# chairclr/PathTracing

Hardware: AMD Instinct MI355X
Metric: Mrays/s (higher is better)
Workload: dtype f32

## Files before the change

pathtracing_amd/csrc/frame.cpp:

```cpp
#include "scene.h"
#include <hip/hip_runtime.h>
#include <algorithm>
#include <cmath>
#include <cstdio>
#include <cstdlib>
#include <cstring>
#include <vector>

using namespace ptrt;

namespace {

uint32_t host_pcg(uint32_t x)
{
    uint32_t s = x * 747796405u + 2891336453u;
    uint32_t w = ((s >> ((s >> 28) + 4u)) ^ s) * 277803737u;
    return (w >> 22) ^ w;
}

uint32_t faster(double rate_simple, double rate_packed) { return rate_packed > 1.10 * rate_simple ? EXT_PACKED : EXT_SIMPLE; }
struct ExtendFrame {
    ExtendChoice &mem;
    bool undecided;
    uint32_t frame_kernel, kernel;
// ... 18 lines not shown
            kernel = EXT_SIMPLE; mixed = probe_n[1] >= enough / 8u;
        } else kernel = mem.kernel = faster(probe_n[0] / std::max((double)ms_simple, 1e-6), probe_n[1] / std::max((double)ms_packed, 1e-6));
        return hipSuccess;
    }
    void frame_done(uint64_t rays, double gpu_ms, bool cold)
    {
        if (!undecided || mem.kernel != 0u || cold) return;
        if (mixed || rays < (1u << 20) || !(gpu_ms > 0.0)) { if (++mem.misses >= 3u) mem.kernel = EXT_SIMPLE; return; }
        (frame_kernel == EXT_PACKED ? mem.rate_packed : mem.rate_simple) = (double)rays / gpu_ms;
        if (mem.rate_simple > 0.0 && mem.rate_packed > 0.0) mem.kernel = faster(mem.rate_simple, mem.rate_packed);
    }
};

hipEvent_t pool_event(pt_context *c, size_t i)
{
    while (c->ev_pool.size() <= i) {
        Event e;
        if (e.create() != hipSuccess) return nullptr;
        c->ev_pool.push_back(std::move(e));
    }
    return c->ev_pool[i];
}

struct Frame {
    uint32_t nranks, streams, pixel_slots, n_slots, shard_cap, samples_per_stream, lag, n_loops, packed_chunk, default_bounces;
    uint32_t forced;
    bool profile, count, split, bucket, full_state, accumulate, mapped, compact;
    bool nee;
    NeeArgs nee_args;
    bool env;
    EnvArgs env_args;
    Accumulation::Key sums_key;
    size_t q_entries; uint64_t total_spp, allocs_before;
    PathState ps; FrameParams fp;
    uint32_t iters; uint64_t slot_launches; size_t n_events;
    std::vector<uint64_t> trace_alive, trace_rays;
};

}

pt_status FrameTemplate::build_if_differs(pt_context *c, hipStream_t q, Key key, const DeviceScene &ds, const PathState &ps, const FrameParams &fp,
                                          const QueueSizes &sizes)
{
    key.q = q_init.p;
    if (valid && key == key_) return PT_OK;
    valid = false; HIP_TRY(c, hipMemsetAsync(cnt_init.p, 0, sizeof(uint32_t) * kCntTotalWords, q));
    PathState pt = ps; pt.counters = cnt_init.p; pt.q_ext[0] = q_init.p;
    const bool dense = key.first_spp < key.streams;
    HIP_TRY(c, launch_generate(q, ds, pt, fp, dense ? 2u : 0u));
    bound = key.shard_cap;
    if (dense) {
        uint32_t *h = sizes.template_sizes();
        HIP_TRY(c, hipMemcpyAsync(h, cnt_init.p, sizeof(uint32_t) * kShards * kCounterStride, hipMemcpyDeviceToHost, q));
        HIP_TRY(c, hipStreamSynchronize(q));
// ... 68 lines not shown
    if (!f.full_state) HIP_TRY(c, c->start.reserve(f.q_entries));
    const uint32_t ovf = s->tree.stack_overflow();
    if (ovf) HIP_TRY(c, c->stack_ovf.ensure((size_t)ovf * f.q_entries));
    if (f.nee) {
        HIP_TRY(c, c->nee_ext.ensure(f.n_slots)); HIP_TRY(c, c->nee_rad.ensure(f.n_slots));
        f.nee_args = NeeArgs{ s->d_lights.p, s->d_cdf.p, s->d_pa.p, s->n_lights, c->nee_ext.p, c->nee_rad.p };
    }
    if (f.env) f.env_args = s->env.args(f.nee && s->env.lit() && s->n_lights ? 0.5f : 1.0f);
    if (f.nranks == 1) HIP_TRY(c, c->out.resize(p->width, p->height));
    PathState &ps = f.ps;
    ps.ray_o = c->ray_o.p; ps.ray_d = c->ray_d.p; ps.thr = c->thr.p; ps.sd = c->sd.p; ps.acc = c->acc.p; ps.q_ext[0] = c->q_ext0.p; ps.q_ext[1] = c->q_ext1.p;
    if (f.split) { ps.hit = c->hit.p; ps.q_bucket[B_METAL] = c->q_metal.p; ps.q_bucket[B_DIELECTRIC] = c->q_dielectric.p; }
    ps.counters = c->counters.p; ps.stack_ovf = c->stack_ovf.p; ps.stack_ovf_entries = ovf; ps.n_slots = f.n_slots; ps.shard_cap = f.shard_cap;
    ps.shard_base = 0; ps.shard_count = kShards; ps.compact_below = t.compact_below; ps.finish_below = t.finish_below; ps.sparse_below = t.sparse_below;
    ps.repack_sticky = (f.samples_per_stream <= t.sticky_samples && t.compact_below > 0.f) ? 1u : 0u;
    ps.host_ring = c->sizes.begin(f.mapped); ps.ring_slots = kLag;
    f.compact = f.bucket || (ps.repack_sticky && f.samples_per_stream <= 2u);
    FrameParams &fp = f.fp;
    fp.width = p->width; fp.height = p->height; fp.spp = p->spp; fp.max_depth = p->max_depth; fp.rr_start = p->rr_start;
    fp.seed_hashed = host_pcg(p->seed); fp.sample_offset = p->sample_offset; fp.ray_eps = p->ray_eps;
    fp.rank = p->rank; fp.nranks = f.nranks; fp.tiles_x = lay.tiles_x; fp.n_tiles = lay.n_tiles; fp.streams = f.streams; fp.slots_per_stream = f.pixel_slots;
    div_magic(f.streams, fp.streams_magic, fp.streams_shift); div_magic(lay.tiles_x, fp.tiles_x_magic, fp.tiles_x_shift);
    fp.offset_mod = p->sample_offset % f.streams; fp.accumulate = f.accumulate ? 1u : 0u;
    return PT_OK;
}

static pt_status start_frame(pt_context *c, const pt_scene *s, const pt_render_params *p, const Frame &f)
{
    hipStream_t q = c->stream;
    if (f.full_state) {
        HIP_TRY(c, hipMemsetAsync(c->counters.p, 0, sizeof(uint32_t) * kCntTotalWords, q));
        HIP_TRY(c, hipEventRecord(c->ev_start, q));
        HIP_TRY(c, launch_generate(q, s->ds, f.ps, f.fp, 1u));
    } else {
        HIP_TRY(c, hipEventRecord(c->ev_start, q));
        FrameTemplate::Key key{};
        key.w = p->width; key.h = p->height; key.rank = p->rank; key.nranks = f.nranks; key.streams = f.streams; key.first_spp = std::min(p->spp, f.streams);
        key.offset = f.fp.offset_mod; key.n_slots = f.n_slots; key.shard_cap = f.shard_cap; key.acc = c->acc.p;
        const pt_status st = c->start.build_if_differs(c, q, key, s->ds, f.ps, f.fp, c->sizes);
        if (st != PT_OK) return st;
        HIP_TRY(c, hipMemcpyAsync(c->counters.p, c->start.counters(), sizeof(uint32_t) * kCntTotalWords, hipMemcpyDeviceToDevice, q));
    }
    c->start.frame_ran(f.accumulate || f.full_state);
    return PT_OK;
}

static pt_status run_loops(pt_context *c, const pt_scene *s, const pt_render_params *p, Frame &f, ExtendFrame &x)
{
    hipStream_t q = c->stream; const uint32_t n_loops = f.n_loops, per_group = kShards / n_loops;
    struct Loop { hipStream_t stream; uint32_t base, bound, iters; bool done; } loops[kMaxGroups];
    HIP_TRY(c, hipEventRecord(c->ev_fork, q));
    for (uint32_t g = 0; g < n_loops; ++g) {
        loops[g] = Loop{ n_loops == 1 ? q : c->group_stream[g], g * per_group, f.full_state ? f.shard_cap : c->start.first_bound(), 0u, false };
        if (loops[g].stream != q) HIP_TRY(c, hipStreamWaitEvent(loops[g].stream, c->ev_fork, 0));
    }
    const uint64_t max_iters = (uint64_t)p->spp * p->max_depth * (f.nee ? 2u : 1u) + kLag + 2;
    const bool trace = f.profile && getenv("PTRT_TRACE") != nullptr;
    const int shade_mode = (s->has_specular || f.env) ? 2 : 0;
    for (uint32_t live = n_loops; live > 0;) {
        for (uint32_t g = 0; g < n_loops; ++g) {
            Loop &L = loops[g];
            if (L.done) continue;
            if (L.iters >= max_iters) return fail(c, PT_ERR_INTERNAL, "wavefront loop did not drain after %u iterations", L.iters);
            const uint32_t it = L.iters; PathState pg = f.ps; pg.shard_base = L.base; pg.shard_count = per_group;
// ... 46 lines not shown
    if (f.nranks == 1)
        HIP_TRY(c, launch_assemble(q, c->out.tiles.p, 1, f.pixel_slots, p->width, p->height, fp.tiles_x, fp.n_tiles, 1.0f / (float)f.total_spp, c->out.fb.p, c->out.fb8.p));
    HIP_TRY(c, hipEventRecord(c->ev_stop, q));
    HIP_TRY(c, hipMemcpyAsync(c->sizes.frame_end(), c->counters.p, sizeof(uint32_t) * kCntTotalWords, hipMemcpyDeviceToHost, q));
    HIP_TRY(c, hipStreamSynchronize(q));
    pt_stats out{}; const CounterView hc{ c->sizes.frame_end(), 0u };
    if (hc.error()) return fail(c, PT_ERR_INTERNAL, "device error flag 0x%x (1 = traversal stack overflow, 2 = step limit)", hc.error());
    for (uint32_t sh = 0; sh < kShards; ++sh) {
        if (hc.word(cnt_alive_index(0, sh)) || hc.word(cnt_alive_index(1, sh)) || hc.word(cnt_alive_index(2, sh))) return fail(c, PT_ERR_INTERNAL, "extend queue of shard %u not empty at frame end", sh);
        out.rays += hc.u64(cnt_rays_index(sh));
    }
    float ms = 0.f; HIP_TRY(c, hipEventElapsedTime(&ms, c->ev_start, c->ev_stop)); out.gpu_ms = ms;
    out.node_visits = hc.u64(kCntNodes); out.tri_tests = hc.u64(kCntTris); out.sphere_tests = hc.u64(kCntSph);
    out.reserved[3] = (hc.u64(kCntWaveNodeIters) & 0xFFFFFFFFFFull) | (hc.u64(kCntWaveNodeIters + 2) << 40);
    if (f.count && getenv("PTRT_TRACE")) {
        const double slots = 64.0 * (double)hc.u64(kCntWaveNodeIters), v = (double)out.node_visits, lf = (double)hc.u64(kCntIdleLeaf), dn = (double)hc.u64(kCntIdleDone);
        if (slots > 0) fprintf(stderr, "ptrt: node-loop lane-slots %.3g: visiting %.1f %%, waiting at a leaf %.1f %%, ray finished %.1f %%, no ray %.1f %%\n", slots,
                               100 * v / slots, 100 * lf / slots, 100 * dn / slots, 100 * (slots - v - lf - dn) / slots);
    }
    out.iterations = f.iters; out.extend_launches = f.iters;
    x.frame_done(out.rays, out.gpu_ms, g_device_allocs != f.allocs_before);
    out.reserved[0] = x.kernel ? x.kernel : (uint32_t)EXT_SIMPLE;
    out.reserved[1] = hc.word(kCntCompactions);
    uint64_t px = 0;
    for (uint32_t t = p->rank; t < fp.n_tiles; t += f.nranks) {
        const uint32_t tx = t % fp.tiles_x, ty = t / fp.tiles_x;
        px += (uint64_t)std::min(kTile, p->width - tx * kTile) * std::min(kTile, p->height - ty * kTile);
    }
    out.paths = px * p->spp;
    out.reserved[2] = f.slot_launches + px * std::min(f.streams, p->spp);
    if (f.profile) {
        const bool trace = getenv("PTRT_TRACE") != nullptr;
        for (size_t i = 0; i + 2 < f.n_events; i += 3) {
            float a = 0.f, b = 0.f; HIP_TRY(c, hipEventElapsedTime(&a, c->ev_pool[i], c->ev_pool[i + 1]));
            HIP_TRY(c, hipEventElapsedTime(&b, c->ev_pool[i + 1], c->ev_pool[i + 2]));
            out.extend_ms += a; out.shade_ms += b;
            if (trace) fprintf(stderr, "ptrt: iteration %3zu  rays %10llu  alive after %10llu  extend %8.3f ms  shade %8.3f ms\n", i / 3,
                               (unsigned long long)(i / 3 < f.trace_rays.size() ? f.trace_rays[i / 3] : 0),
                               (unsigned long long)(i / 3 < f.trace_alive.size() ? f.trace_alive[i / 3] : 0), a, b);
        }
        out.other_ms = out.gpu_ms - out.extend_ms - out.shade_ms;
    }
    c->out.tiles_hold(f.pixel_slots); c->sums.complete(f.sums_key, f.total_spp);
    if (f.nranks == 1) c->out.complete(FrameOutputs::Holds::path_traced);
    if (stats) *stats = out;
    return PT_OK;
}

static pt_status render_frame(pt_context *c, const pt_scene *s, const pt_render_params *p, pt_stats *stats)
{
    if (!c || !p) return fail(c, PT_ERR_INVALID_ARGUMENT, "pt_render: NULL argument");
    pt_tile_layout lay; pt_status st = layout_of(p, &lay);
    if (st != PT_OK) return fail(c, st, "pt_render: bad width/height/rank/nranks/tile_size");
    HIP_TRY(c, hipSetDevice(c->device));
    c->out.replace();
    if (p->mode == PT_REFERENCE_SPHERE) {
        HIP_TRY(c, c->out.resize(p->width, p->height));
        HIP_TRY(c, hipEventRecord(c->ev_start, c->stream));
        HIP_TRY(c, launch_reference_sphere(c->stream, p->width, p->height, c->out.fb.p, c->out.fb8.p));
        HIP_TRY(c, hipEventRecord(c->ev_stop, c->stream));
        HIP_TRY(c, hipStreamSynchronize(c->stream));
        float ms = 0.f; HIP_TRY(c, hipEventElapsedTime(&ms, c->ev_start, c->ev_stop));
        pt_stats out{};
        out.gpu_ms = ms; out.other_ms = ms; out.rays = out.paths = (uint64_t)p->width * p->height; out.iterations = 1;
// ... 19 lines not shown
```

pathtracing_amd/csrc/kernels.hip:

```cpp
#include "ptrt_internal.h"
#include "pt_device.h"
#include <algorithm>
#include <cstdlib>
#include <type_traits>


using namespace ptd;

namespace ptrt {

PT_DEV uint32_t lane_prefix(uint64_t m) { return __builtin_amdgcn_mbcnt_hi((uint32_t)(m >> 32), __builtin_amdgcn_mbcnt_lo((uint32_t)m, 0u)); }
PT_DEV uint32_t lane_id() { return lane_prefix(~0ull); }

typedef const float4 __attribute__((address_space(4))) *uniform_f4;
PT_DEV uniform_f4 as_uniform(const float4 *p) { return (uniform_f4)(uintptr_t)p; }
PT_DEV float4 uniform_load(uniform_f4 p, uint32_t i) { return make_float4(p[i].x, p[i].y, p[i].z, p[i].w); }
PT_DEV uint32_t spheres_test(const float4 *spheres, uint32_t n_spheres, uint32_t first_id, V3 o, V3 d, Hit &h)
{
    const uniform_f4 sp = as_uniform(spheres);
    for (uint32_t j = 0; j < n_spheres; j += 4u) {
        const float4 s0 = uniform_load(sp, j), s1 = uniform_load(sp, j + 1u), s2 = uniform_load(sp, j + 2u), s3 = uniform_load(sp, j + 3u);
        sphere_test(s0, first_id + j, o, d, h);
        if (j + 1u < n_spheres) sphere_test(s1, first_id + j + 1u, o, d, h);
        if (j + 2u < n_spheres) sphere_test(s2, first_id + j + 2u, o, d, h);
// ... 352 lines not shown
}
PT_DEV void path_init(const DeviceScene &sc, const FrameParams &fp, uint32_t slot, PathRegs &r)
{
    uint32_t x = 0, y = 0;
    slot_pixel(slot, fp, x, y);
    r.sample = first_sample(slot, fp);
    r.key = path_key(fp.seed_hashed, y * fp.width + x, fp.sample_offset + r.sample);
    camera_ray_of(sc.cam, x, y, r.key, r.o, r.d);
    r.T = v3(1.f, 1.f, 1.f);
    r.depth = 0u;
}
template <bool NEE = false>
PT_DEV void path_begin(uint32_t it, uint32_t slot, PathRegs &r, NeeRegs *nr = nullptr)
{
    if (it == 0u) {
        path_init(cold().sc, cold().fp, slot, r);
        if (!cold().fp.accumulate) at(cold().ps.acc, slot) = make_float4(0.f, 0.f, 0.f, 0.f);
    } else {
        const PathState &ps = cold().ps;
        path_load(ps, slot, r);
        if constexpr (NEE) { nr->flags = __float_as_uint(at(ps.ray_o, slot).w); nr->aux = at(ps.ray_d, slot).w; }
    }
}

__global__ void __launch_bounds__(kBlock) k_generate(DeviceScene sc, PathState ps, FrameParams fp, uint32_t full)
{
    uint32_t shard, bx, nbx;
    block_pos(ps, shard, bx, nbx);
    const uint32_t j = bx * kBlock + threadIdx.x;
    const uint32_t t = j >> kShardGroupShift, rot = (shard + kShards - t % kShards) % kShards;
    const uint32_t slot = ((t * kShards + rot) << kShardGroupShift) | (j & ((1u << kShardGroupShift) - 1u));
    uint32_t x = 0, y = 0;
    const bool in_range = j < ps.shard_cap && slot < ps.n_slots;
    const uint32_t first = first_sample(slot, fp);
    const bool valid = in_range && first < fp.spp && slot_pixel(slot, fp, x, y);
    if (in_range && !fp.accumulate) ps.acc[slot] = make_float4(0.f, 0.f, 0.f, 0.f);
    if (valid && full == 1u) {
        PathRegs r;
        path_init(sc, fp, slot, r);
        path_store(ps, slot, r);
    }
    if (full == 2u) wave_push(&ps.counters[cnt_ext_index(0, shard)], ps.q_ext[0] + (size_t)shard * ps.shard_cap, valid, slot);
    else if (j < ps.shard_cap) ps.q_ext[0][(size_t)shard * ps.shard_cap + j] = valid ? slot : kInvalidSlot;
    const uint32_t n_alive = (uint32_t)__syncthreads_count(valid);
    if (threadIdx.x == 0) {
        if (n_alive) atomicAdd(&ps.counters[cnt_alive_index(0, shard)], n_alive);
        if (bx == 0 && full != 2u) ps.counters[cnt_ext_index(0, shard)] = ps.shard_cap;
    }
}


PT_DEV bool next_sample(const DeviceScene &sc, const FrameParams &fp, uint32_t slot, PathRegs &r, uint32_t &depth)
{
    uint32_t &key = r.key, &sample = r.sample;
    bool alive = false;
    sample += fp.streams;
    if (sample < fp.spp) {
        uint32_t x = 0, y = 0;
        slot_pixel(slot, fp, x, y);
        key = path_key(fp.seed_hashed, y * fp.width + x, fp.sample_offset + sample);
        camera_ray_of(sc.cam, x, y, key, r.o, r.d);
        r.T = v3(1.f, 1.f, 1.f);
        depth = 0;
        alive = true;
    }
    return alive;
}

template <int MODE, bool NEE = false, bool ENV = false>
PT_DEV bool shade_one(const DeviceScene &sc, const PathState &ps, const FrameParams &fp, uint32_t slot, PathRegs &r, float t, uint32_t ref,
                      uint32_t b, uint32_t &defer, NeeRegs *nr = nullptr)
// ... 472 lines not shown
    return h;
}

template <int L, bool COUNT, int FUSE, bool NEE = false, bool ENV = false>
__global__ void __launch_bounds__(kExtBlock) __attribute__((amdgpu_waves_per_eu(PT_EXT_WAVES_FOR(L, FUSE, NEE, ENV), PT_EXT_WAVES_FOR(L, FUSE, NEE, ENV))))
k_extend(typename ExtArgsFor<NEE, ENV>::type a)
{
    static_assert(!NEE || (FUSE != SHADE_NONE && !COUNT), "NEE: fused shading, no visit counters");
    static_assert(!ENV || (FUSE == SHADE_INLINE && !COUNT), "ENV: all-kinds fused shading, no visit counters");
    const HotScene g = hot_scene(a.sc);
    const uint32_t it = a.it;
    __shared__ int32_t s_stack[kStackLds * kExtBlock];
    __shared__ uint32_t s_stash[(FUSE != SHADE_NONE ? (NEE ? 7 : 5) : 1) * kExtBlock];
    const uint32_t tid = threadIdx.x;
    ExtHead hd;
    uint32_t gid, qbase, slot = kInvalidSlot, n_bounces;
    {
        const PathState &ps = cold().ps;
        hd = extend_head<FUSE>(a, ps, kExtBlock, tid, true, false);
        gid = hd.bx * kExtBlock + tid;
        if (hd.idle) return;
        qbase = hd.shard * ps.shard_cap;
        if (gid < hd.n) slot = at(ps.q_ext[hd.parity], qbase + gid);
        const bool sparse = hd.do_compact && (float)hd.n_alive < ps.sparse_below * (float)hd.n;
        n_bounces = FUSE == SHADE_NONE ? 1u : (hd.n_alive <= ps.finish_below ? kFinishVertices : sparse ? 1u : a.bounces);
    }
    const uint32_t shard = hd.shard, parity = hd.parity, n = hd.n;
    const bool active = slot != kInvalidSlot;
    const StackCtx stk{ s_stack, kExtBlock, tid, qbase + gid };

    VisitCounts vc;
    __shared__ int32_t s_state[COUNT ? 64 : 1];
    PathRegs r;
    r.o = v3(0.f, 0.f, 0.f); r.d = v3(0.f, 0.f, 1.f); r.T = v3(0.f, 0.f, 0.f); r.key = r.sample = r.depth = 0u;
    NeeRegs nr{ 0.0f, 0u };
    if (active) {
        if (FUSE == SHADE_NONE) { const PathState &ps = cold().ps; r.o = xyz(at(ps.ray_o, slot)); r.d = xyz(at(ps.ray_d, slot)); }
        else path_begin<NEE>(it, slot, r, &nr);
    }
    bool alive = active;
    uint32_t wave_rays = 0;
    for (uint32_t bounce = 0; bounce < n_bounces; ++bounce) {
    const uint64_t alive_mask = __ballot(alive);
    if (alive_mask == 0) break;
    wave_rays += (uint32_t)__popcll(alive_mask);
    if (COUNT && kExtBlock == 64u) { s_state[tid] = alive ? 0 : 1; __syncthreads(); }
// ... 92 lines not shown
            } else {
                stash_restore(s_stash, 64u, lane, r);
                uint32_t defer = 0u;
                const bool alive = shade_one<FUSE>(cold().sc, cold().ps, cold().fp, slot, r, h.t, h.ref, B_LAMBERT, defer);
                --budget;
                if (alive && budget != 0u) start_ray();
                else {
                    if (alive) path_store(cold().ps, slot, r);
                    retired = true; retire_alive = alive; has = false;
                }
            }
        }
        if (FUSE != SHADE_NONE) {
            wave_rays += (uint32_t)__popcll(__ballot(fin && has));
            wave_alive += (uint32_t)__popcll(__ballot(retire_alive));
            if (do_compact) wave_push(&cold().ps.counters[cnt_ext_index(hd.cnext, shard)], q_next, retire_alive, slot);
            else if (retired) q_next[pos] = retire_alive ? slot : kInvalidSlot;
        }
        const uint64_t idle = __ballot(!has);
        const uint32_t avail = end - next;
        if (idle && avail) {
            const uint32_t prefix = lane_prefix(idle);
            const bool pull = !has && prefix < avail;
            if (pull) { pos = next + prefix; slot = queue[pos]; }
            if (pull && slot == kInvalidSlot) {
                if (FUSE != SHADE_NONE && !do_compact) q_next[pos] = kInvalidSlot;
            } else if (pull) {
                if (FUSE == SHADE_NONE) { o = xyz(at(cold().ps.ray_o, slot)); d = xyz(at(cold().ps.ray_d, slot)); }
                else path_begin(it, slot, r);
                budget = budget0;
                start_ray();
                has = true;
            }
            if (FUSE != SHADE_NONE) wave_rays += (uint32_t)__popcll(__ballot(pull && has));
            next += min((uint32_t)__popcll(idle), avail);
        }
        if (!__ballot(has)) {
            if (next < end) continue;
            break;
        }
        const uint32_t want = (next < end) ? kRefillIdle : 64u;
        for (;;) {
            if (cur != PT_BVH_EMPTY) {
                const bool inner = cur >= 0;
                const uint32_t enc = (uint32_t)~cur, first = enc >> 3, more = enc & 7u;
                const float4 *base = inner ? nodes + (size_t)cur * node_rows<L>() : tris + (size_t)first * 4;
                const float4 r0 = base[0], r1 = base[1], r2 = base[2], r3 = base[3];
// ... 286 lines not shown
    const float4 a = gathered[(size_t)rank * slots_per_rank + ((size_t)tl << (2 * kTileShift)) + inner];
    const float4 c = make_float4(a.x * inv_spp, a.y * inv_spp, a.z * inv_spp, a.w * inv_spp);
    const size_t i = (size_t)y * width + x;
    fb[i] = c;
    fb8[i] = unorm8(c.x) | (unorm8(c.y) << 8) | (unorm8(c.z) << 16) | (unorm8(c.w) << 24);
    (void)n_tiles;
}

static inline uint32_t blocks_for(uint32_t n) { return n ? (n + kBlock - 1) / kBlock : 1u; }

hipError_t launch_reference_sphere(hipStream_t s, uint32_t w, uint32_t h, float4 *out_f, uint32_t *out8)
{
    dim3 block(64, 4, 1), grid((w + 63) / 64, (h + 3) / 4, 1);
    hipLaunchKernelGGL(k_reference_sphere, grid, block, 0, s, w, h, out_f, out8);
    return hipGetLastError();
}

hipError_t launch_generate(hipStream_t s, const DeviceScene &sc, const PathState &ps, const FrameParams &fp, uint32_t mode)
{
    hipLaunchKernelGGL(k_generate, shard_grid(blocks_for(ps.shard_cap), ps.shard_count), dim3(kBlock), 0, s, sc, ps, fp, mode);
    return hipGetLastError();
}

template <typename F>
static bool with_layout(uint32_t width, F &&f)
{
    switch (width) {
    case PT_BVH_WIDTH_2: f(std::integral_constant<int, PT_BVH_WIDTH_2>{}); return true;
    case PT_BVH_WIDTH_4: f(std::integral_constant<int, PT_BVH_WIDTH_4>{}); return true;
    case PT_BVH_WIDTH_4Q: f(std::integral_constant<int, PT_BVH_WIDTH_4Q>{}); return true;
    case PT_BVH_WIDTH_8Q: f(std::integral_constant<int, PT_BVH_WIDTH_8Q>{}); return true;
    case PT_BVH_WIDTH_8O: f(std::integral_constant<int, PT_BVH_WIDTH_8O>{}); return true;
    default: return false;
    }
}
template <typename F>
static void with_fuse(int fuse, F &&f)
{
    if (fuse == SHADE_QUEUE) f(std::integral_constant<int, SHADE_QUEUE>{});
    else if (fuse == SHADE_INLINE) f(std::integral_constant<int, SHADE_INLINE>{});
    else f(std::integral_constant<int, SHADE_NONE>{});
}

hipError_t launch_extend(hipStream_t s, const DeviceScene &sc, const PathState &ps, const FrameParams &fp, uint32_t it, uint32_t shard_bound, bool count,
                         int kernel, uint32_t packed_chunk, int fuse, bool compact, uint32_t bounces, const NeeArgs *nee, const EnvArgs *env)
{
// ... 82 lines not shown
```

pathtracing_amd/csrc/ptrt_internal.h:

```cpp
#pragma once
#include <hip/hip_runtime_api.h>
#include <stdint.h>
#include "../../include/ptrt.h"

namespace ptrt {

constexpr uint32_t kTileShift = 6;
constexpr uint32_t kTile = 1u << kTileShift;
constexpr uint32_t kTilePixels = kTile * kTile;
constexpr uint32_t kBlock = 256;
#ifndef PT_SHARD_GROUP_SHIFT
#define PT_SHARD_GROUP_SHIFT 6
#endif
constexpr uint32_t kShardGroupShift = PT_SHARD_GROUP_SHIFT;
#ifndef PT_STACK_LDS
#define PT_STACK_LDS 12
#endif
#ifndef PT_EXT_BLOCK
#define PT_EXT_BLOCK 64
#endif
constexpr uint32_t kStackLds = PT_STACK_LDS;
constexpr uint32_t kExtBlock = PT_EXT_BLOCK;
constexpr uint32_t kMaxSpheres = 64;
constexpr uint32_t kTraceBlocks = 16384;
// ... 73 lines not shown
    float4 *ext;
    float4 *rad;
};

struct EnvArgs {
    const float4 *texels;
    const float *mcdf;
    const float *ccdf;
    uint32_t n;
    float nf, step;
    uint32_t lit;
    float psel;
};

struct FrameParams {
    uint32_t width, height, spp, max_depth, rr_start, seed_hashed, sample_offset;
    float ray_eps;
    uint32_t rank, nranks, tiles_x, n_tiles;
    uint32_t streams;
    uint32_t slots_per_stream;
    uint32_t accumulate;
    uint32_t streams_magic, streams_shift, tiles_x_magic, tiles_x_shift;
    uint32_t offset_mod;
};
inline void div_magic(uint32_t d, uint32_t &magic, uint32_t &shift)
{
    if (d <= 1u) { magic = 0u; shift = 0u; return; }
    uint32_t l = 0; while ((1ull << l) < d) ++l;
    magic = (uint32_t)(((1ull << (31u + l)) + d - 1u) / d); shift = l - 1u;
}
inline __host__ __device__ uint32_t div_by(uint32_t n, uint32_t magic, uint32_t shift)
{
    return magic ? (uint32_t)(((uint64_t)n * magic) >> 32) >> shift : n;
}

hipError_t launch_reference_sphere(hipStream_t s, uint32_t w, uint32_t h, float4 *out_f, uint32_t *out_rgba8);
hipError_t launch_generate(hipStream_t s, const DeviceScene &sc, const PathState &ps, const FrameParams &fp, uint32_t mode);
hipError_t launch_extend(hipStream_t s, const DeviceScene &sc, const PathState &ps, const FrameParams &fp, uint32_t it, uint32_t shard_bound, bool count,
                         int kernel, uint32_t packed_chunk, int fuse, bool compact, uint32_t bounces, const NeeArgs *nee = nullptr,
                         const EnvArgs *env = nullptr);
hipError_t launch_shade(hipStream_t s, const DeviceScene &sc, const PathState &ps, const FrameParams &fp, uint32_t it, uint32_t shard_bound, int mode, bool compact);
uint32_t trace_blocks(uint32_t n);
hipError_t launch_trace(hipStream_t s, const DeviceScene &sc, const PathState &ps, const float4 *rays, float4 *hits, uint32_t n, bool occlusion, bool count);
hipError_t launch_reduce_streams(hipStream_t s, const float4 *acc, float4 *tiles, uint32_t slots_per_stream, uint32_t streams);
hipError_t launch_assemble(hipStream_t s, const float4 *gathered, uint32_t nranks, uint32_t slots_per_rank,
                           uint32_t width, uint32_t height, uint32_t tiles_x, uint32_t n_tiles, float inv_spp,
                           float4 *fb, uint32_t *fb8);

int context_device(const pt_context *c);
hipStream_t context_stream(const pt_context *c);
void context_set_error(pt_context *c, const char *msg);

struct BinaryBvh;
struct DeviceBlob4Q;
hipError_t build_lbvh_device(hipStream_t s, const float *verts9, uint32_t n_tris, BinaryBvh &out);
hipError_t build_lbvh_blob4q_device(hipStream_t s, const float *verts9, const uint32_t *mats, uint32_t n_tris, DeviceBlob4Q &out);

}
```

pathtracing_amd/csrc/scene.cpp:

```cpp
#include "scene.h"
#include "refit.h"
#include <hip/hip_runtime.h>
#include <algorithm>
#include <atomic>
#include <chrono>
#include <cmath>
#include <cstdio>
#include <cstdlib>
#include <cstring>
#include <new>

using namespace ptrt;


struct ptrt::CommitClock {
    std::chrono::steady_clock::time_point t = std::chrono::steady_clock::now();
    void lap(const char *what)
    {
        static const bool timing = getenv("PTRT_TIMING") != nullptr;
        if (timing) fprintf(stderr, "ptrt commit: %-28s %8.2f ms\n", what, std::chrono::duration<double, std::milli>(std::chrono::steady_clock::now() - t).count());
        t = std::chrono::steady_clock::now();
    }
};

void CommittedTree::adopt(BvhBlob &&blob, uint32_t layout_id)
{
    layout = layout_id; fan = blob.width; n_nodes = blob.n_nodes; n_tris = (uint32_t)blob.tris.size();
    max_depth = blob.max_depth; stack_need = blob.stack_need; sah_cost = blob.sah_cost; build_ms = blob.build_ms;
    packed.clear();
    if (layout_quantised(layout)) {
        if (fan == 4) quantize_bvh4(blob, packed);
        else quantize_bvh8(blob, packed);
    }
    slots = std::move(blob.slots); tris = std::move(blob.tris);
    node_bytes = layout_quantised(layout) ? packed.size() : slots.size() * sizeof(BvhSlot);
    image = Image::fresh; upload_pending = true;
}

void CommittedTree::adopt(DeviceBlob4Q &&blob, uint32_t n_records)
{
    d_nodes = std::move(blob.nodes); d_tris = std::move(blob.tris);
    layout = PT_BVH_WIDTH_4Q; fan = layout_fan(layout); n_nodes = blob.n_nodes; n_tris = n_records;
    max_depth = blob.max_depth; stack_need = blob.stack_need; sah_cost = blob.sah_cost; build_ms = blob.device_ms;
    node_bytes = (uint64_t)n_nodes * layout_node_bytes(layout);
    slots.clear(); packed.clear(); tris.clear();
    image = Image::absent; upload_pending = false;
}

pt_status CommittedTree::upload(pt_context *c, CommitClock &clock)
{
    if (node_bytes > (1ull << 32) || (uint64_t)n_tris * 64u > (1ull << 32))
        return fail(c, PT_ERR_UNSUPPORTED, "BVH of %llu node bytes and %llu triangle records: each array must stay within 4 GiB",
                    (unsigned long long)node_bytes, (unsigned long long)n_tris);
    HIP_TRY(c, hipSetDevice(context_device(c)));
    static_assert(sizeof(BvhSlot) == 32 && sizeof(BvhTri) == 48 && sizeof(pt_material) == 48, "blob layout");
    if (!upload_pending) return PT_OK;
    HIP_TRY(c, d_nodes.ensure((size_t)(node_bytes / 16)));
    HIP_TRY(c, d_tris.ensure(tris.size() * 4));
    std::vector<float> rec(tris.size() * 16);
    for (size_t i = 0; i < tris.size(); ++i) {
        const BvhTri &t = tris[i];
        std::memcpy(&rec[i * 16], &t, sizeof(BvhTri));
        shading_row(t.e1, t.e2, t.mat, &rec[i * 16 + 12]);
    }
    clock.lap("triangle records");
    if (!rec.empty()) HIP_TRY(c, hipMemcpy(d_tris.p, rec.data(), rec.size() * sizeof(float), hipMemcpyHostToDevice));
    clock.lap("upload triangles");
    if (node_bytes) HIP_TRY(c, hipMemcpy(d_nodes.p, node_data(), node_bytes, hipMemcpyHostToDevice));
    upload_pending = false;
// ... 17 lines not shown
    return PT_OK;
}

pt_status CommittedTree::refs(pt_context *c, std::vector<int32_t> &out) const
{
    const uint32_t stride = layout_node_bytes(layout);
    out.resize((size_t)n_nodes * fan);
    if (image == Image::absent) {
        if (n_nodes) HIP_TRY(c, hipMemcpy2D(out.data(), 4 * fan, (const uint8_t *)d_nodes.p + layout_ref_at(layout, 0), stride, 4 * fan, n_nodes, hipMemcpyDeviceToHost));
        return PT_OK;
    }
    const uint8_t *nd = (const uint8_t *)node_data();
    for (size_t i = 0; i < n_nodes; ++i)
        for (uint32_t k = 0; k < fan; ++k) std::memcpy(&out[i * fan + k], nd + i * stride + layout_ref_at(layout, k), 4);
    return PT_OK;
}

pt_status CommittedTree::ids(pt_context *c, std::vector<uint32_t> &out) const
{
    out.resize(n_tris);
    if (image == Image::absent) { if (n_tris) HIP_TRY(c, hipMemcpy2D(out.data(), 4, (const uint8_t *)d_tris.p + 12, 64, 4, n_tris, hipMemcpyDeviceToHost)); }
    else for (uint32_t j = 0; j < n_tris; ++j) out[j] = tris[j].id;
    return PT_OK;
}

pt_status SceneVertices::host(pt_context *c, const float *&verts9)
{
    if (host_stale) {
        HIP_TRY(c, hipSetDevice(context_device(c)));
        HIP_TRY(c, hipMemcpy(host_.data(), dev[cur].p, host_.size() * sizeof(float), hipMemcpyDeviceToHost));
        host_stale = false;
    }
    verts9 = host_.data();
    return PT_OK;
}

pt_status SceneVertices::device(pt_context *c, const float *&verts9) const
{
    if (!dev_current) {
        HIP_TRY(c, hipSetDevice(context_device(c)));
        HIP_TRY(c, dev[cur].ensure(host_.size()));
        if (!host_.empty()) HIP_TRY(c, hipMemcpy(dev[cur].p, host_.data(), host_.size() * sizeof(float), hipMemcpyHostToDevice));
        dev_current = true;
    }
    verts9 = dev[cur].p;
    return PT_OK;
// ... 238 lines not shown
    DeviceScene &d = s->ds;
    d.nodes = s->tree.d_nodes.p; d.tris = s->tree.d_tris.p; d.spheres = s->d_spheres.p; d.sph_mat = s->d_sph_mat.p; d.mats = s->d_mats.p;
    d.n_nodes = s->tree.n_nodes; d.n_tris = (uint32_t)s->tri_mat.size(); d.n_spheres = (uint32_t)s->sph_mat.size(); d.n_mats = (uint32_t)s->mats.size();
    for (int k = 0; k < 3; ++k) d.sky[k] = s->sky[k];
    d.bvh_width = s->tree.layout;
    d.cam = s->cam;
    s->has_specular = false;
    for (const pt_material &m : s->mats) if (m.kind != PT_LAMBERT) s->has_specular = true;
    s->committed = true;
}

pt_status pt_scene_commit(pt_scene *s, uint32_t bvh_width)
{
    if (!s) return fail(nullptr, PT_ERR_INVALID_ARGUMENT, "scene is NULL");
    bool lbvh = false;
    pt_status st = check_commit(s, bvh_width, lbvh);
    if (st != PT_OK) return st;
    CommitClock clock;
    s->serial = next_scene_serial(); s->updates = 0;
    s->cache.invalidate();
    if ((st = build_tree(s, bvh_width, lbvh, clock)) != PT_OK) return st;
    if (!s->ctx) { s->committed = true; return PT_OK; }
    if ((st = s->tree.upload(s->ctx, clock)) != PT_OK || (st = upload_primitives(s, clock)) != PT_OK || (st = light_table(s, clock)) != PT_OK) return st;
    publish_scene(s);
    return PT_OK;
}

pt_status pt_scene_bvh_info(const pt_scene *s, pt_bvh_info *o)
{
    if (!s || !o) return fail(s ? s->ctx : nullptr, PT_ERR_INVALID_ARGUMENT, "NULL argument");
    if (!s->committed) return fail(s->ctx, PT_ERR_NOT_COMMITTED, "scene not committed");
    std::memset(o, 0, sizeof *o);
    const CommittedTree &t = s->tree;
    o->width = t.layout; o->n_nodes = t.n_nodes; o->n_tris = t.n_tris;
    o->max_depth = t.max_depth;
    o->node_bytes = t.node_bytes;
    o->tri_bytes = (uint64_t)t.n_tris * sizeof(BvhTri);
    o->build_ms = t.build_ms; o->sah_cost = t.sah_cost;
    o->stack_need = t.stack_need;
    return PT_OK;
}

pt_status pt_scene_bvh_read(const pt_scene *s, void *nodes, uint64_t node_bytes, void *tris48, uint64_t tri_bytes)
{
    if (!s) return fail(nullptr, PT_ERR_INVALID_ARGUMENT, "scene is NULL");
    if (!s->committed) return fail(s->ctx, PT_ERR_NOT_COMMITTED, "scene not committed");
// ... 53 lines not shown
        if ((st = check_device_array(c, verts9, count * 36u, "verts9", "pt_scene_update_triangles", "PT_UPDATE_HOST_MEMORY")) != PT_OK) return st;
    }
    auto &R = s->cache.refit;
    if (!R.ready && (st = prepare_refit(s)) != PT_OK) return st;
    hipStream_t q = context_stream(c);
    const CommittedTree &tree = s->tree;
    float *v = s->verts.next();
    if (host) HIP_TRY(c, hipMemcpyAsync(v, verts9, count * 36u, hipMemcpyHostToDevice, q));
    HIP_TRY(c, hipEventRecord(R.ev[0], q));
    float ms_check = 0.f;
    if (!host) {
        HIP_TRY(c, hipMemsetAsync(R.flag.p, 0, sizeof(uint32_t), q));
        HIP_TRY(c, launch_refit_stage(q, (const float *)verts9, v, count * 9u, R.flag.p));
        HIP_TRY(c, hipEventRecord(R.ev[1], q));
        uint32_t bad = 0;
        HIP_TRY(c, hipMemcpyAsync(&bad, R.flag.p, sizeof bad, hipMemcpyDeviceToHost, q));
        HIP_TRY(c, hipStreamSynchronize(q));
        if (bad) return fail(c, PT_ERR_INVALID_ARGUMENT, "pt_scene_update_triangles: non-finite vertex coordinate in the device array");
        HIP_TRY(c, hipEventElapsedTime(&ms_check, R.ev[0], R.ev[1]));
        HIP_TRY(c, hipEventRecord(R.ev[0], q));
    }
    const uint32_t layout = tree.layout;
    ++s->updates;
    HIP_TRY(c, launch_refit_tris(q, v, tree.d_tris.p, tree.n_tris, R.tbox.p));
    for (size_t l = 0; l + 1 < R.level_off.size(); ++l)
        HIP_TRY(c, launch_refit_level(q, layout, tree.d_nodes.p, R.list.p + R.level_off[l], R.level_off[l + 1] - R.level_off[l], R.tbox.p, R.nbox.p, R.carea.p));
    const uint32_t nb = refit_sah_blocks(tree.n_nodes);
    HIP_TRY(c, launch_refit_sah(q, layout, tree.d_nodes.p, tree.n_nodes, R.carea.p, R.nbox.p, R.sah.p, R.sah.p + nb));
    HIP_TRY(c, hipEventRecord(R.ev[2], q));
    double sah = 0.0;
    HIP_TRY(c, hipMemcpyAsync(&sah, R.sah.p + nb, sizeof sah, hipMemcpyDeviceToHost, q));
    HIP_TRY(c, hipStreamSynchronize(q));
    float ms = 0.f;
    HIP_TRY(c, hipEventElapsedTime(&ms, R.ev[0], R.ev[2]));
    out.gpu_ms = (double)ms + ms_check;
    if (!s->pa_span.empty()) {
        const uint32_t lo = s->light_cand.front(), hi = s->light_cand.back();
        std::vector<float> span(host ? 0u : (size_t)(hi - lo + 1u) * 9u);
        if (!host) HIP_TRY(c, hipMemcpy(span.data(), v + (size_t)lo * 9u, span.size() * sizeof(float), hipMemcpyDeviceToHost));
        if ((st = host ? build_lights(c, s, (const float *)verts9, 0) : build_lights(c, s, span.data(), lo)) != PT_OK) return st;
    }
    s->verts.next_is_current();
    s->tree.device_rewritten((float)sah);
    if (stats) *stats = out;
    return PT_OK;
}

static pt_status update_spheres(pt_scene *s, const float *cxyzr, uint64_t count)
{
    if (!s) return fail(nullptr, PT_ERR_INVALID_ARGUMENT, "pt_scene_update_spheres: scene is NULL");
    pt_context *c = s->ctx;
    if (!s->committed) return fail(c, PT_ERR_NOT_COMMITTED, "pt_scene_update_spheres: scene not committed");
    const uint64_t ns = s->sph_mat.size();
    if (count != ns) return fail(c, PT_ERR_INVALID_ARGUMENT, "pt_scene_update_spheres: count %llu, the scene was committed with %llu spheres", (unsigned long long)count, (unsigned long long)ns);
    if (count && !cxyzr) return fail(c, PT_ERR_INVALID_ARGUMENT, "pt_scene_update_spheres: cxyzr is NULL");
// ... 46 lines not shown
```

pathtracing_amd/csrc/scene.h:

```cpp
#pragma once
#include "context.h"
#include "bvh_build.h"
#include "blob_rules.h"
#include "environment.h"
#include <vector>

namespace ptrt {

struct CommitClock;

uint64_t next_scene_serial();

class CommittedTree {
public:
    DevBuf<float4> d_nodes, d_tris;
    uint32_t layout = 0, fan = 0;
    uint32_t n_nodes = 0, n_tris = 0;
    uint32_t max_depth = 0, stack_need = 0;
    float sah_cost = 0.f;
    double build_ms = 0.0;
    uint64_t node_bytes = 0;
    uint32_t stack_overflow() const { return stack_need > kStackLds ? stack_need - kStackLds : 0u; }

    void adopt(BvhBlob &&blob, uint32_t layout_id);
    void adopt(DeviceBlob4Q &&blob, uint32_t n_records);
    pt_status upload(pt_context *c, CommitClock &clock);
    void device_rewritten(float new_sah_cost) { sah_cost = new_sah_cost; if (image == Image::fresh) image = Image::topology_only; }
    pt_status host_image(pt_context *c, const void *&nodes, const BvhTri *&tris) const;
    pt_status refs(pt_context *c, std::vector<int32_t> &out) const;
    pt_status ids(pt_context *c, std::vector<uint32_t> &out) const;

private:
    enum class Image { fresh, topology_only, absent };
    mutable Image image = Image::fresh;
    mutable std::vector<BvhSlot> slots;
    mutable std::vector<uint8_t> packed;
    mutable std::vector<BvhTri> tris;
    bool upload_pending = false;
    const void *node_data() const { return layout_quantised(layout) ? (const void *)packed.data() : (const void *)slots.data(); }
};

class SceneVertices {
public:
    void set(const float *verts9, uint64_t count) { host_.assign(verts9, verts9 + count * 9); host_stale = false; dev_current = false; }
    pt_status host(pt_context *c, const float *&verts9);
    pt_status device(pt_context *c, const float *&verts9) const;
    hipError_t reserve_device()
    {
        const hipError_t e = dev[0].ensure(host_.size());
        return e != hipSuccess ? e : dev[1].ensure(host_.size());
    }
    float *next() const { return dev[cur ^ 1u].p; }
    void next_is_current() { cur ^= 1u; host_stale = true; dev_current = true; }

private:
// ... 57 lines not shown
```

Before: 17340.

## Resolve primary rays that miss the projected scene bounds at frame start

Projects the BVH root box, widened to cover the spheres, onto the camera image to get a conservative pixel rectangle that can contain geometry. Pixels outside that rectangle get the sky colour from a small kernel at frame start. The first-iteration extend and shade kernels drop those slots from the queue, so their primary rays are never traversed. Those untraced rays are still added to the reported ray count. The root bound is fetched to the host after commit and refit, which adds a synchronous copy, and the rectangle must stay conservative for the image to remain correct.

```diff
diff --git a/pathtracing_amd/csrc/frame.cpp b/pathtracing_amd/csrc/frame.cpp
--- a/pathtracing_amd/csrc/frame.cpp
+++ b/pathtracing_amd/csrc/frame.cpp
@@ -64,6 +64,48 @@
     return c->ev_pool[i];
 }
 
+bool scene_pixels(const pt_scene *s, const pt_camera &cam, uint32_t W, uint32_t H, FrameParams &fp)
+{
+    fp.scene_x0 = fp.scene_y0 = 0u; fp.scene_x1 = fp.scene_y1 = ~0u;
+    Box tb;
+    if (!s->tree.root_bound(tb)) return false;
+    double lo[3], hi[3], o[3], big = 0.0;
+    for (int k = 0; k < 3; ++k) { lo[k] = tb.lo[k]; hi[k] = tb.hi[k]; o[k] = cam.origin[k]; big = std::max(big, std::fabs(o[k])); }
+    for (size_t i = 0; i < s->sph_mat.size(); ++i) {
+        const float *sp = &s->spheres[i * 4];
+        const double r = sp[3], dx = sp[0] - o[0], dy = sp[1] - o[1], dz = sp[2] - o[2], reach = std::sqrt(dx * dx + dy * dy + dz * dz) + r;
+        const double rr = std::sqrt(r * r + std::ldexp(reach * reach, -16));
+        for (int k = 0; k < 3; ++k) { lo[k] = std::min(lo[k], sp[k] - rr); hi[k] = std::max(hi[k], sp[k] + rr); }
+    }
+    if (!(lo[0] <= hi[0])) { fp.scene_x0 = fp.scene_x1 = fp.scene_y0 = fp.scene_y1 = ~0u; return true; }
+    for (int k = 0; k < 3; ++k) big = std::max(big, std::max(std::fabs(lo[k]), std::fabs(hi[k])));
+    if (!(big < 1e15)) return false;
+    for (int k = 0; k < 3; ++k) { lo[k] -= 1e-4 * big; hi[k] += 1e-4 * big; }
+    const double R[3] = { cam.right[0], cam.right[1], cam.right[2] }, U[3] = { cam.up[0], cam.up[1], cam.up[2] }, F[3] = { cam.forward[0], cam.forward[1], cam.forward[2] };
+    auto cross = [](const double *a, const double *b, double *c) { c[0] = a[1] * b[2] - a[2] * b[1]; c[1] = a[2] * b[0] - a[0] * b[2]; c[2] = a[0] * b[1] - a[1] * b[0]; };
+    auto dot = [](const double *a, const double *b) { return a[0] * b[0] + a[1] * b[1] + a[2] * b[2]; };
+    double UF[3], FR[3], RU[3];
+    cross(U, F, UF); cross(F, R, FR); cross(R, U, RU);
+    const double det = dot(R, UF), scale = cam.scale;
+    if (!(std::fabs(det) > 1e-6 * std::sqrt(dot(R, R) * dot(U, U) * dot(F, F))) || !(scale > 0.0) || !std::isfinite(scale)) return false;
+    double x0 = INFINITY, x1 = -INFINITY, y0 = INFINITY, y1 = -INFINITY;
+    for (int i = 0; i < 8; ++i) {
+        const double v[3] = { ((i & 1) ? hi[0] : lo[0]) - o[0], ((i & 2) ? hi[1] : lo[1]) - o[1], ((i & 4) ? hi[2] : lo[2]) - o[2] };
+        const double a = dot(v, UF) / det, b = dot(v, FR) / det, c = dot(v, RU) / det;
+        if (!(c > 1e-4 * (std::fabs(a) + std::fabs(b) + std::fabs(c)))) return false;
+        const double px = (a / c + cam.cx) / scale, py = (b / c + cam.cy) / scale;
+        x0 = std::min(x0, px); x1 = std::max(x1, px); y0 = std::min(y0, py); y1 = std::max(y1, py);
+    }
+    const double mx = 1.0 + 1e-4 * ((double)W + std::fabs(cam.cx / scale)), my = 1.0 + 1e-4 * ((double)H + std::fabs(cam.cy / scale));
+    x0 -= mx; x1 += mx; y0 -= my; y1 += my;
+    if (!std::isfinite(x0) || !std::isfinite(x1) || !std::isfinite(y0) || !std::isfinite(y1)) return false;
+    auto px_of = [](double v, uint32_t n) { return (uint32_t)std::min(std::max(v, 0.0), (double)n); };
+    fp.scene_x0 = px_of(std::floor(x0), W); fp.scene_x1 = px_of(std::ceil(x1), W);
+    fp.scene_y0 = px_of(std::floor(y0), H); fp.scene_y1 = px_of(std::ceil(y1), H);
+    if (fp.scene_x0 == 0u && fp.scene_x1 >= W && fp.scene_y0 == 0u && fp.scene_y1 >= H) { fp.scene_x1 = fp.scene_y1 = ~0u; return false; }
+    return true;
+}
+
 struct Frame {
     uint32_t nranks, streams, pixel_slots, n_slots, shard_cap, samples_per_stream, lag, n_loops, packed_chunk, default_bounces;
     uint32_t forced;
@@ -72,6 +114,7 @@
     NeeArgs nee_args;
     bool env;
     EnvArgs env_args;
+    bool sky;
     Accumulation::Key sums_key;
     size_t q_entries; uint64_t total_spp, allocs_before;
     PathState ps; FrameParams fp;
@@ -186,6 +229,8 @@
     fp.rank = p->rank; fp.nranks = f.nranks; fp.tiles_x = lay.tiles_x; fp.n_tiles = lay.n_tiles; fp.streams = f.streams; fp.slots_per_stream = f.pixel_slots;
     div_magic(f.streams, fp.streams_magic, fp.streams_shift); div_magic(lay.tiles_x, fp.tiles_x_magic, fp.tiles_x_shift);
     fp.offset_mod = p->sample_offset % f.streams; fp.accumulate = f.accumulate ? 1u : 0u;
+    fp.scene_x0 = fp.scene_y0 = 0u; fp.scene_x1 = fp.scene_y1 = ~0u;
+    f.sky = !f.full_state && !f.count && !f.env && scene_pixels(s, s->ds.cam, p->width, p->height, fp);
     return PT_OK;
 }
 
@@ -204,6 +249,7 @@
         const pt_status st = c->start.build_if_differs(c, q, key, s->ds, f.ps, f.fp, c->sizes);
         if (st != PT_OK) return st;
         HIP_TRY(c, hipMemcpyAsync(c->counters.p, c->start.counters(), sizeof(uint32_t) * kCntTotalWords, hipMemcpyDeviceToDevice, q));
+        if (f.sky) HIP_TRY(c, launch_sky_pixels(q, s->ds, f.ps, f.fp));
     }
     c->start.frame_ran(f.accumulate || f.full_state);
     return PT_OK;
@@ -296,12 +342,16 @@
     x.frame_done(out.rays, out.gpu_ms, g_device_allocs != f.allocs_before);
     out.reserved[0] = x.kernel ? x.kernel : (uint32_t)EXT_SIMPLE;
     out.reserved[1] = hc.word(kCntCompactions);
-    uint64_t px = 0;
+    uint64_t px = 0, scene_px = 0;
     for (uint32_t t = p->rank; t < fp.n_tiles; t += f.nranks) {
         const uint32_t tx = t % fp.tiles_x, ty = t / fp.tiles_x;
-        px += (uint64_t)std::min(kTile, p->width - tx * kTile) * std::min(kTile, p->height - ty * kTile);
+        const uint32_t xa = tx * kTile, ya = ty * kTile, xb = xa + std::min(kTile, p->width - xa), yb = ya + std::min(kTile, p->height - ya);
+        px += (uint64_t)(xb - xa) * (yb - ya);
+        const int64_t ix = (int64_t)std::min(xb, fp.scene_x1) - (int64_t)std::max(xa, fp.scene_x0), iy = (int64_t)std::min(yb, fp.scene_y1) - (int64_t)std::max(ya, fp.scene_y0);
+        scene_px += (uint64_t)(std::max<int64_t>(ix, 0) * std::max<int64_t>(iy, 0));
     }
     out.paths = px * p->spp;
+    out.rays += (px - scene_px) * p->spp;
     out.reserved[2] = f.slot_launches + px * std::min(f.streams, p->spp);
     if (f.profile) {
         const bool trace = getenv("PTRT_TRACE") != nullptr;
@@ -314,6 +364,8 @@
                                (unsigned long long)(i / 3 < f.trace_alive.size() ? f.trace_alive[i / 3] : 0), a, b);
         }
         out.other_ms = out.gpu_ms - out.extend_ms - out.shade_ms;
+        if (trace && f.sky) fprintf(stderr, "ptrt: sky pixels x [%u, %u) y [%u, %u) excepted: %llu of %llu pixels, %llu rays resolved at frame start\n", fp.scene_x0,
+                                    fp.scene_x1, fp.scene_y0, fp.scene_y1, (unsigned long long)(px - scene_px), (unsigned long long)px, (unsigned long long)((px - scene_px) * p->spp));
     }
     c->out.tiles_hold(f.pixel_slots); c->sums.complete(f.sums_key, f.total_spp);
     if (f.nranks == 1) c->out.complete(FrameOutputs::Holds::path_traced);
diff --git a/pathtracing_amd/csrc/kernels.hip b/pathtracing_amd/csrc/kernels.hip
--- a/pathtracing_amd/csrc/kernels.hip
+++ b/pathtracing_amd/csrc/kernels.hip
@@ -398,6 +398,15 @@
         if constexpr (NEE) { nr->flags = __float_as_uint(at(ps.ray_o, slot).w); nr->aux = at(ps.ray_d, slot).w; }
     }
 }
+PT_DEV uint32_t queued_slot(uint32_t it, uint32_t slot)
+{
+    if (it == 0u && slot != kInvalidSlot) {
+        uint32_t x = 0, y = 0;
+        slot_pixel(slot, cold().fp, x, y);
+        if (sky_pixel(cold().fp, x, y)) slot = kInvalidSlot;
+    }
+    return slot;
+}
 
 __global__ void __launch_bounds__(kBlock) k_generate(DeviceScene sc, PathState ps, FrameParams fp, uint32_t full)
 {
@@ -423,6 +432,21 @@
         if (n_alive) atomicAdd(&ps.counters[cnt_alive_index(0, shard)], n_alive);
         if (bx == 0 && full != 2u) ps.counters[cnt_ext_index(0, shard)] = ps.shard_cap;
     }
+}
+
+__global__ void __launch_bounds__(kBlock) k_sky_pixels(DeviceScene sc, PathState ps, FrameParams fp)
+{
+    const uint32_t slot = blockIdx.x * kBlock + threadIdx.x;
+    uint32_t x = 0, y = 0;
+    if (slot >= ps.n_slots || !slot_pixel(slot, fp, x, y) || !sky_pixel(fp, x, y)) return;
+    const uint32_t first = first_sample(slot, fp);
+    if (first >= fp.spp) return;
+    float4 A = fp.accumulate ? ps.acc[slot] : make_float4(0.f, 0.f, 0.f, 0.f);
+    for (uint32_t s = first; s < fp.spp; s += fp.streams) {
+        A.x = fma_(1.0f, sc.sky[0], A.x); A.y = fma_(1.0f, sc.sky[1], A.y); A.z = fma_(1.0f, sc.sky[2], A.z);
+        A.w += 1.0f;
+    }
+    ps.acc[slot] = A;
 }
 
 
@@ -941,6 +965,7 @@
         if (hd.idle) return;
         qbase = hd.shard * ps.shard_cap;
         if (gid < hd.n) slot = at(ps.q_ext[hd.parity], qbase + gid);
+        if (FUSE != SHADE_NONE) slot = queued_slot(it, slot);
         const bool sparse = hd.do_compact && (float)hd.n_alive < ps.sparse_below * (float)hd.n;
         n_bounces = FUSE == SHADE_NONE ? 1u : (hd.n_alive <= ps.finish_below ? kFinishVertices : sparse ? 1u : a.bounces);
     }
@@ -1079,7 +1104,7 @@
         if (idle && avail) {
             const uint32_t prefix = lane_prefix(idle);
             const bool pull = !has && prefix < avail;
-            if (pull) { pos = next + prefix; slot = queue[pos]; }
+            if (pull) { pos = next + prefix; slot = queue[pos]; if (FUSE != SHADE_NONE) slot = queued_slot(it, slot); }
             if (pull && slot == kInvalidSlot) {
                 if (FUSE != SHADE_NONE && !do_compact) q_next[pos] = kInvalidSlot;
             } else if (pull) {
@@ -1412,6 +1437,12 @@
     return hipGetLastError();
 }
 
+hipError_t launch_sky_pixels(hipStream_t s, const DeviceScene &sc, const PathState &ps, const FrameParams &fp)
+{
+    hipLaunchKernelGGL(k_sky_pixels, dim3(blocks_for(ps.n_slots)), dim3(kBlock), 0, s, sc, ps, fp);
+    return hipGetLastError();
+}
+
 template <typename F>
 static bool with_layout(uint32_t width, F &&f)
 {
diff --git a/pathtracing_amd/csrc/ptrt_internal.h b/pathtracing_amd/csrc/ptrt_internal.h
--- a/pathtracing_amd/csrc/ptrt_internal.h
+++ b/pathtracing_amd/csrc/ptrt_internal.h
@@ -119,7 +119,12 @@
     uint32_t accumulate;
     uint32_t streams_magic, streams_shift, tiles_x_magic, tiles_x_shift;
     uint32_t offset_mod;
+    uint32_t scene_x0, scene_x1, scene_y0, scene_y1;
 };
+inline __host__ __device__ bool sky_pixel(const FrameParams &fp, uint32_t x, uint32_t y)
+{
+    return x < fp.scene_x0 || x >= fp.scene_x1 || y < fp.scene_y0 || y >= fp.scene_y1;
+}
 inline void div_magic(uint32_t d, uint32_t &magic, uint32_t &shift)
 {
     if (d <= 1u) { magic = 0u; shift = 0u; return; }
@@ -133,6 +138,7 @@
 
 hipError_t launch_reference_sphere(hipStream_t s, uint32_t w, uint32_t h, float4 *out_f, uint32_t *out_rgba8);
 hipError_t launch_generate(hipStream_t s, const DeviceScene &sc, const PathState &ps, const FrameParams &fp, uint32_t mode);
+hipError_t launch_sky_pixels(hipStream_t s, const DeviceScene &sc, const PathState &ps, const FrameParams &fp);
 hipError_t launch_extend(hipStream_t s, const DeviceScene &sc, const PathState &ps, const FrameParams &fp, uint32_t it, uint32_t shard_bound, bool count,
                          int kernel, uint32_t packed_chunk, int fuse, bool compact, uint32_t bounces, const NeeArgs *nee = nullptr,
                          const EnvArgs *env = nullptr);
diff --git a/pathtracing_amd/csrc/scene.cpp b/pathtracing_amd/csrc/scene.cpp
--- a/pathtracing_amd/csrc/scene.cpp
+++ b/pathtracing_amd/csrc/scene.cpp
@@ -34,7 +34,7 @@
     }
     slots = std::move(blob.slots); tris = std::move(blob.tris);
     node_bytes = layout_quantised(layout) ? packed.size() : slots.size() * sizeof(BvhSlot);
-    image = Image::fresh; upload_pending = true;
+    image = Image::fresh; upload_pending = true; bound_valid = false;
 }
 
 void CommittedTree::adopt(DeviceBlob4Q &&blob, uint32_t n_records)
@@ -44,7 +44,7 @@
     max_depth = blob.max_depth; stack_need = blob.stack_need; sah_cost = blob.sah_cost; build_ms = blob.device_ms;
     node_bytes = (uint64_t)n_nodes * layout_node_bytes(layout);
     slots.clear(); packed.clear(); tris.clear();
-    image = Image::absent; upload_pending = false;
+    image = Image::absent; upload_pending = false; bound_valid = false;
 }
 
 pt_status CommittedTree::upload(pt_context *c, CommitClock &clock)
@@ -108,6 +108,40 @@
     if (image == Image::absent) { if (n_tris) HIP_TRY(c, hipMemcpy2D(out.data(), 4, (const uint8_t *)d_tris.p + 12, 64, 4, n_tris, hipMemcpyDeviceToHost)); }
     else for (uint32_t j = 0; j < n_tris; ++j) out[j] = tris[j].id;
     return PT_OK;
+}
+
+hipError_t CommittedTree::fetch_root(hipStream_t q)
+{
+    if (!n_nodes) return hipSuccess;
+    if (layout_node_bytes(layout) > sizeof root_bytes) return hipErrorInvalidValue;
+    return hipMemcpyAsync(root_bytes, d_nodes.p, layout_node_bytes(layout), hipMemcpyDeviceToHost, q);
+}
+
+void CommittedTree::root_fetched()
+{
+    bound = Box::empty();
+    if (n_nodes) {
+        uint32_t w[sizeof root_bytes / 4];
+        std::memcpy(w, root_bytes, sizeof root_bytes);
+        for (uint32_t c = 0; c < fan; ++c) {
+            int32_t ref; std::memcpy(&ref, root_bytes + layout_ref_at(layout, c), 4);
+            if (ref == kEmptyRef) continue;
+            Box b;
+            if (layout_quantised(layout)) {
+                const uint32_t kw = fan / 4u, q0 = 4u + fan;
+                for (uint32_t a = 0; a < 3; ++a) {
+                    const float org = bits_as_float(w[a]), sc = quant_scale_of((w[3] >> (8u * a)) & 0xffu);
+                    const uint32_t ql = (w[q0 + kw * a + c / 4u] >> (8u * (c % 4u))) & 0xffu, qh = (w[q0 + kw * (3u + a) + c / 4u] >> (8u * (c % 4u))) & 0xffu;
+                    b.lo[a] = __builtin_fmaf((float)ql, sc, org); b.hi[a] = __builtin_fmaf((float)qh, sc, org);
+                }
+            } else {
+                BvhSlot sl; std::memcpy(&sl, root_bytes + 32u * c, sizeof sl);
+                for (int a = 0; a < 3; ++a) { b.lo[a] = sl.lo[a]; b.hi[a] = sl.hi[a]; }
+            }
+            bound.grow(b);
+        }
+    }
+    bound_valid = true;
 }
 
 pt_status SceneVertices::host(pt_context *c, const float *&verts9)
@@ -392,6 +426,8 @@
     if ((st = build_tree(s, bvh_width, lbvh, clock)) != PT_OK) return st;
     if (!s->ctx) { s->committed = true; return PT_OK; }
     if ((st = s->tree.upload(s->ctx, clock)) != PT_OK || (st = upload_primitives(s, clock)) != PT_OK || (st = light_table(s, clock)) != PT_OK) return st;
+    HIP_TRY(s->ctx, s->tree.fetch_root(context_stream(s->ctx))); HIP_TRY(s->ctx, hipStreamSynchronize(context_stream(s->ctx)));
+    s->tree.root_fetched();
     publish_scene(s);
     return PT_OK;
 }
@@ -491,6 +527,7 @@
     }
     const uint32_t layout = tree.layout;
     ++s->updates;
+    s->tree.bound_stale();
     HIP_TRY(c, launch_refit_tris(q, v, tree.d_tris.p, tree.n_tris, R.tbox.p));
     for (size_t l = 0; l + 1 < R.level_off.size(); ++l)
         HIP_TRY(c, launch_refit_level(q, layout, tree.d_nodes.p, R.list.p + R.level_off[l], R.level_off[l + 1] - R.level_off[l], R.tbox.p, R.nbox.p, R.carea.p));
@@ -499,7 +536,9 @@
     HIP_TRY(c, hipEventRecord(R.ev[2], q));
     double sah = 0.0;
     HIP_TRY(c, hipMemcpyAsync(&sah, R.sah.p + nb, sizeof sah, hipMemcpyDeviceToHost, q));
+    HIP_TRY(c, s->tree.fetch_root(q));
     HIP_TRY(c, hipStreamSynchronize(q));
+    s->tree.root_fetched();
     float ms = 0.f;
     HIP_TRY(c, hipEventElapsedTime(&ms, R.ev[0], R.ev[2]));
     out.gpu_ms = (double)ms + ms_check;
diff --git a/pathtracing_amd/csrc/scene.h b/pathtracing_amd/csrc/scene.h
--- a/pathtracing_amd/csrc/scene.h
+++ b/pathtracing_amd/csrc/scene.h
@@ -29,8 +29,15 @@
     pt_status host_image(pt_context *c, const void *&nodes, const BvhTri *&tris) const;
     pt_status refs(pt_context *c, std::vector<int32_t> &out) const;
     pt_status ids(pt_context *c, std::vector<uint32_t> &out) const;
+    void bound_stale() { bound_valid = false; }
+    hipError_t fetch_root(hipStream_t q);
+    void root_fetched();
+    bool root_bound(Box &out) const { out = bound; return bound_valid; }
 
 private:
+    Box bound = Box::empty();
+    bool bound_valid = false;
+    uint8_t root_bytes[256] = {};
     enum class Image { fresh, topology_only, absent };
     mutable Image image = Image::fresh;
     mutable std::vector<BvhSlot> slots;
```

Result: faster. 17730, median of 6 (+2.2%).
